# facebookresearch/AudioDec

Hardware: AMD Instinct MI355X
Metric: 48 kHz hop-300 frames/s/GPU + per-frame encode+decode latency (ms) (higher is better)
Workload: dtype f32 (conv operands split into f16 hi + lo/2048 pairs, 3 f16 MFMAs per product sum, f32 accumulate)

## Files before the change

### audiodec_amd/csrc/adk_common.h

```cpp
#pragma once
#include <hip/hip_runtime.h>
#include <stdint.h>
#include <string>
#include <algorithm>
#include <cstring>
#include <initializer_list>
#include "../../include/audiodec_hip.h"

namespace adk {

void set_error(const std::string& msg);
int fail(int code, const std::string& msg);

inline int check_pointers(const std::string& f, const char* names, bool missing, std::initializer_list<const void*> ptrs) {
    if (missing) return fail(ADK_ERR_ARG, f + ": null pointer");
    uintptr_t bits = 0;
    for (const void* p : ptrs) bits |= reinterpret_cast<uintptr_t>(p);
    if (bits & 3) return fail(ADK_ERR_ARG, f + ": " + names + " must be 4-byte aligned");
    return ADK_OK;
}

#define ADK_HIP_CHECK(expr)                                                                   \
    do {                                                                                      \
        hipError_t _e = (expr);                                                               \
        if (_e != hipSuccess)                                                                 \
            return ::adk::fail(ADK_ERR_HIP, std::string(#expr) + ": " + hipGetErrorString(_e)); \
    } while (0)

struct ConvArgs {
    const float* in;   int in_rows, in_ch, in_row0, in_choff, in_gstride;
    float* out;        int out_rows, out_ch, out_cursor, out_choff;
    const float* res;  int res_rows, res_ch, res_cursor, res_choff, res_gstride;
    const float* w;    const float* wfrag;  const float* bias;
    int cin_g, cout_g, groups, taps, stride, dilation, up, cout_real;
    int act_in, act_out; float slope;
    int batch, t_out, n_total;
    int ktot;
    int* err = nullptr;
    const float* in_sh = nullptr;
    float* out_sh = nullptr;
    int sh_act = 0; float sh_slope = 0.f;
};
inline int* conv_err_word(const ConvArgs& a);

__device__ __forceinline__ float expm1_neg(float x) {
    const float q = fmaf(fmaf(fmaf(fmaf(fmaf(1.f / 5040.f, x, 1.f / 720.f), x, 1.f / 120.f), x, 1.f / 24.f), x, 1.f / 6.f), x, 0.5f);
    const float p = fmaf(x * x, q, x);
    const float e = __builtin_amdgcn_exp2f(x * 1.44269504088896341f) - 1.0f;
    return x > -0.4f ? p : e;
}

__device__ __forceinline__ float act_apply(float x, int act, float slope) {
    if (act == ADK_ACT_ELU) return x > 0.f ? x : expm1_neg(x);
    if (act == ADK_ACT_LEAKY) return x > 0.f ? x : x * slope;
    if (act == ADK_ACT_TANH) return tanhf(x);
    return x;
}

__device__ __forceinline__ float rvq_residual_step(float& r, float q) {
    const float qp = __fadd_rn(r, __fsub_rn(q, r));
    r = __fsub_rn(r, qp);
    return qp;
}

struct RingMeanArgs {
    const float* src[4]; int src_rows[4], src_cursor[4];
    float* out; int out_rows, out_cursor;
    int n, channels, batch, t;
};
int launch_ring_mean(const RingMeanArgs& m, hipStream_t s);
int launch_hist_replicate(float* ring, int rows, int channels, int cursor, int hist, int batch, hipStream_t s);
int launch_conv_direct(const ConvArgs& a, hipStream_t s);
bool conv_cin1_write_ok(const ConvArgs& a);
int launch_conv_cin1_write(const ConvArgs& a, const float* src, hipStream_t s);
struct Workspace { float* ptr = nullptr; size_t bytes = 0; size_t flags_offset = 0; unsigned epoch = 0;
                   int workgroups = 0; };
int launch_conv_mfma(const ConvArgs& a, hipStream_t s, Workspace& ws);
size_t conv_mfma_workspace_bytes(size_t* flags_offset);
bool conv_rl_supported(const ConvArgs& a);
bool conv_rl_preferred(const ConvArgs& a);
int launch_conv_rl(const ConvArgs& a, hipStream_t s);
bool conv_rl16_supported(const ConvArgs& a);
bool conv_rl16_preferred(const ConvArgs& a);
int launch_conv_rl16(const ConvArgs& a, hipStream_t s);
bool conv_rl16_fusable(const ConvArgs& a1, const ConvArgs& a2);
int launch_conv_rl16_fused(const ConvArgs& a1, const ConvArgs& a2, hipStream_t s);
bool conv_rb16_fusable(const ConvArgs* c, int n);
int launch_conv_rb16(const ConvArgs* c, int n, const int* keep, hipStream_t s);
const char* conv_rb16_name(const ConvArgs* c, int n);
bool conv_ou16_fusable(const ConvArgs& a1, const ConvArgs& a2);
int launch_conv_ou16(const ConvArgs& a1, const ConvArgs& a2, hipStream_t s);
bool conv_oc16_fusable(const ConvArgs& a1, const ConvArgs& a2);
int launch_conv_oc16(const ConvArgs& a1, const ConvArgs& a2, hipStream_t s);
bool conv_up16_supported(const ConvArgs& a);
int launch_conv_up16(const ConvArgs& a, hipStream_t s);
int launch_conv_sk16(const ConvArgs& a, hipStream_t s, Workspace& ws);
int conv_sk16_pick(const ConvArgs& a);
bool conv_gv16_preferred(const ConvArgs& a);
int conv_set_option(const char* name, int value);
int rvq_set_option(const char* name, int value);
int rvq_ema_set_option(const char* name, int value);
int launch_pack_split16(const float* w, float* out, int groups, int cout_g, int ktot, hipStream_t s);
int* flags_word();
inline int* conv_err_word(const ConvArgs& a) { return a.err ? a.err : flags_word(); }
constexpr int kMaxDevices = 64;
int flag_pool_acquire(int device, int** word);
void flag_pool_release(int device, int* word);
int flag_pool_fetch(int device, int* word, hipStream_t s, int* v);
int flag_pool_take(int device, int* word, int* v);
int flag_pool_fetch_all(int device, int* acc);
inline int current_device() { int d = 0; (void)hipGetDevice(&d); return (d >= 0 && d < kMaxDevices) ? d : 0; }
inline int device_of(const void* ptr) {
    hipPointerAttribute_t at;
    if (ptr && hipPointerGetAttributes(&at, ptr) == hipSuccess && at.type == hipMemoryTypeDevice && at.device >= 0 && at.device < kMaxDevices)
        return at.device;
    (void)hipGetLastError();
    return current_device();
}
struct DeviceGuard {
    int prev = -1;
    explicit DeviceGuard(int device) {
        int cur = -1;
        if (hipGetDevice(&cur) == hipSuccess && cur != device) { if (hipSetDevice(device) == hipSuccess) prev = cur; }
    }
    ~DeviceGuard() { if (prev >= 0) (void)hipSetDevice(prev); }
};
int launch_pack_weights(const float* w, float* out, int groups, int cout_g, int ktot, hipStream_t s);
bool conv_mfma_supported(const ConvArgs& a);
int conv_mfma_pick(const ConvArgs& a);
const char* conv_mfma_cfg_name(int pick);
bool conv_mfma_force_cfg(int cfg);
int streamk_plan(long long tiles, int nchunks, int cap, int out[4]);
long long streamk_range_start(long long tiles, int nchunks, const int plan[4], int r);

}
```

### audiodec_amd/csrc/conv_mfma.hip

```cpp
#include "conv_split16.h"
#include <cstring>
#include <atomic>

#ifndef ADK_SK_SC1_READ
#define ADK_SK_SC1_READ 1
#endif
#ifndef ADK_SK_OWNER_LATE
#define ADK_SK_OWNER_LATE 1
#endif
#ifndef ADK_SK16_DBG
#define ADK_SK16_DBG 0
#endif

namespace adk {

#if ADK_SK16_DBG & 32
__device__ unsigned long long g_sk_wg_trace[512 * 4];
#endif
#if ADK_SK16_DBG & 16
__device__ unsigned long long g_sk_trace[64 * 8];
#define SK_STAMP(slot) do { if (trace_on && it < 64) { __builtin_amdgcn_sched_barrier(0); const unsigned long long t_ = __builtin_amdgcn_s_memtime(); \
                            __builtin_amdgcn_sched_barrier(0); if (lane == 0) trace_lds[it * 8 + (slot)] = t_; } } while (0)
#else
#define SK_STAMP(slot) do { } while (0)
#endif

constexpr int KC = 64;
constexpr int kGvCounters = 4096;

struct SkArgs {
    float* ws;
    unsigned* flags;
    unsigned epoch;
    int G;
    int split;
    int owner_chunks;
    int tpw;
    int tiles;
    int m_tiles, n_tiles, nchunks;
    int cpt;
    int kgroups;
    int mt32_per_g;
    unsigned in_bytes, w_bytes;
    unsigned ws_bytes;
    int* err;
    float inv_t_out;
    long long total;
    int epi_lds;
};

constexpr int kActPre = 100;

__host__ __device__ __forceinline__ long long sk_range_start(int r, int G, int split, int tpw, int tiles, int nchunks, int owner_chunks, long long total) {
    if (split > 0) {
        const int t = r / split, p = r - t * split;
        if (split == 2) return (long long)t * nchunks + (p ? owner_chunks : 0);
        return (long long)t * nchunks + (p * nchunks) / split;
    }
    if (tpw > 0) {
        long long t = (long long)r * tpw;
        if (t > tiles) t = tiles;
        return t * nchunks;
    }
    return (long long)r * total / G;
}
__device__ __forceinline__ long long sk_u0(int r, const SkArgs& sk) {
    return sk_range_start(r, sk.G, sk.split, sk.tpw, sk.tiles, sk.nchunks, sk.owner_chunks, sk.total);
}

template <int NJ, bool CHECK = false>
__device__ __forceinline__ void sk_epilogue(const ConvArgs& a, const f32x16 (&acc)[NJ], int g, int ml0, int n0w, int lane, int* err = nullptr) {
    const int l31 = lane & 31, lh = lane >> 5;
    bool bad = false;
#pragma unroll
    for (int j = 0; j < NJ; ++j) {
        const int n = n0w + j * 32 + l31;
        if (n >= a.n_total) continue;
        const int b = n / a.t_out, t = n - b * a.t_out;
        const float* resp = nullptr;
        if (a.res) {
            int rrow = a.res_cursor + t;
            if (rrow >= a.res_rows) rrow -= a.res_rows;
            resp = a.res + ((size_t)b * a.res_rows + rrow) * a.res_ch + a.res_choff + g * a.res_gstride;
        }
        float* outb = a.out + (size_t)b * a.out_rows * a.out_ch + a.out_choff;
        const int obase = a.out_cursor + t * a.up;
#pragma unroll
        for (int qd = 0; qd < 4; ++qd) {
            const int ml = ml0 + 8 * qd + 4 * lh;
            if (ml >= a.cout_g) continue;
            const int mg = g * a.cout_g + ml;
            float4 v = make_float4(acc[j][4 * qd], acc[j][4 * qd + 1], acc[j][4 * qd + 2], acc[j][4 * qd + 3]);
            if (CHECK) bad |= not_finite4(v);
            if (a.bias) {
                const float4 bb = *reinterpret_cast<const float4*>(a.bias + mg);
                v.x += bb.x; v.y += bb.y; v.z += bb.z; v.w += bb.w;
            }
            if (resp) {
                const float4 rr = *reinterpret_cast<const float4*>(resp + ml);
                v.x += rr.x; v.y += rr.y; v.z += rr.z; v.w += rr.w;
            }
            if (a.act_out != ADK_ACT_NONE) {
                v.x = act_apply(v.x, a.act_out, 0.f); v.y = act_apply(v.y, a.act_out, 0.f);
                v.z = act_apply(v.z, a.act_out, 0.f); v.w = act_apply(v.w, a.act_out, 0.f);
            }
            int orow = obase, ocol = mg;
            if (a.up > 1) { const int ph = mg / a.cout_real; orow += ph; ocol = mg - ph * a.cout_real; }
            if (orow >= a.out_rows) orow -= a.out_rows;
            *reinterpret_cast<float4*>(outb + (size_t)orow * a.out_ch + ocol) = v;
            if (CHECK && a.out_sh) {
                const float x[4] = {act_apply(v.x, a.sh_act, a.sh_slope), act_apply(v.y, a.sh_act, a.sh_slope),
                                    act_apply(v.z, a.sh_act, a.sh_slope), act_apply(v.w, a.sh_act, a.sh_slope)};
                f16x4 hi, lo;
#pragma unroll
                for (int e = 0; e < 4; ++e) split_to(x[e], hi, lo, e);
                unsigned char* srow = reinterpret_cast<unsigned char*>(a.out_sh + ((size_t)b * a.out_rows + orow) * a.out_ch + a.out_choff);
                unsigned char* sp = srow + (size_t)(ocol >> 3) * 32 + (ocol & 4) * 2;
                *reinterpret_cast<f16x4*>(sp) = hi;
                *reinterpret_cast<f16x4*>(sp + 16) = lo;
            }
        }
    }
    if (CHECK && bad) atomicOr(err, 8);
}

__device__ __forceinline__ void sk_tile_coords(int tile, const SkArgs& sk, int& g, int& mt, int& nt) {
    mt = tile % sk.m_tiles;
    const int rest = tile / sk.m_tiles;
    nt = rest % sk.n_tiles;
    g = rest / sk.n_tiles;
}

__device__ __forceinline__ int fast_div(int n, int d, float inv_d) {
    int q = (int)(__int2float_rn(n) * inv_d);
    int r = n - q * d;
    if (r < 0) { --q; r += d; }
    if (r >= d) { ++q; }
    return q;
}

template <int NJ, int BM, int BN, int NT, bool CHECK>
__device__ __forceinline__ void sk_epilogue_lds(const ConvArgs& a, const f32x16 (&acc)[NJ], float* T, int g, int m0, int n0, int wm, int wn,
                                                int tid, float inv_t_out, int* err) {
    constexpr int TSF = BM + 4;
    const int lane = tid & 63, l31 = lane & 31, lh = lane >> 5;
#pragma unroll
    for (int j = 0; j < NJ; ++j) {
        float* trow = T + (size_t)(wn * NJ * 32 + j * 32 + l31) * TSF + wm * 32 + 4 * lh;
#pragma unroll
        for (int qd = 0; qd < 4; ++qd)
            *reinterpret_cast<float4*>(trow + 8 * qd) = make_float4(acc[j][4 * qd], acc[j][4 * qd + 1], acc[j][4 * qd + 2], acc[j][4 * qd + 3]);
    }
    __syncthreads();
    constexpr int GPC = BM / 8;
    bool bad = false;
    for (int it = tid; it < BN * GPC; it += NT) {
        const int col = it / GPC, cg = it - col * GPC;
        const int n = n0 + col;
        const int ml = m0 + 8 * cg;
        if (n >= a.n_total || ml >= a.cout_g) continue;
        float4 t0 = *reinterpret_cast<const float4*>(T + (size_t)col * TSF + 8 * cg);
        float4 t1 = *reinterpret_cast<const float4*>(T + (size_t)col * TSF + 8 * cg + 4);
        if (CHECK) bad |= not_finite(t0.x) | not_finite(t0.y) | not_finite(t0.z) | not_finite(t0.w) |
                          not_finite(t1.x) | not_finite(t1.y) | not_finite(t1.z) | not_finite(t1.w);
        const int b = fast_div(n, a.t_out, inv_t_out), t = n - b * a.t_out;
        const int mg = g * a.cout_g + ml;
        if (a.bias) {
            const float4 b0 = *reinterpret_cast<const float4*>(a.bias + mg), b1 = *reinterpret_cast<const float4*>(a.bias + mg + 4);
            t0.x += b0.x; t0.y += b0.y; t0.z += b0.z; t0.w += b0.w;
            t1.x += b1.x; t1.y += b1.y; t1.z += b1.z; t1.w += b1.w;
        }
        if (a.res) {
            int rrow = a.res_cursor + t;
            if (rrow >= a.res_rows) rrow -= a.res_rows;
            const float* resp = a.res + ((size_t)b * a.res_rows + rrow) * a.res_ch + a.res_choff + g * a.res_gstride + ml;
            const float4 r0 = *reinterpret_cast<const float4*>(resp), r1 = *reinterpret_cast<const float4*>(resp + 4);
            t0.x += r0.x; t0.y += r0.y; t0.z += r0.z; t0.w += r0.w;
            t1.x += r1.x; t1.y += r1.y; t1.z += r1.z; t1.w += r1.w;
        }
        float x[8] = {t0.x, t0.y, t0.z, t0.w, t1.x, t1.y, t1.z, t1.w};
        if (a.act_out != ADK_ACT_NONE) {
#pragma unroll
            for (int e = 0; e < 8; ++e) x[e] = act_apply(x[e], a.act_out, 0.f);
        }
        int orow = a.out_cursor + t * a.up, ocol = mg;
        if (a.up > 1) { const int ph = mg / a.cout_real; orow += ph; ocol = mg - ph * a.cout_real; }
        if (orow >= a.out_rows) orow -= a.out_rows;
        const size_t oidx = ((size_t)b * a.out_rows + orow) * a.out_ch + a.out_choff + ocol;
        *reinterpret_cast<float4*>(a.out + oidx) = make_float4(x[0], x[1], x[2], x[3]);
        *reinterpret_cast<float4*>(a.out + oidx + 4) = make_float4(x[4], x[5], x[6], x[7]);
        if (CHECK && a.out_sh) {
            f16x8 hi, lo;
#pragma unroll
            for (int e = 0; e < 8; ++e) split_to(act_apply(x[e], a.sh_act, a.sh_slope), hi, lo, e);
            unsigned char* sp = reinterpret_cast<unsigned char*>(a.out_sh + ((size_t)b * a.out_rows + orow) * a.out_ch + a.out_choff) + (size_t)(ocol >> 3) * 32;
            *reinterpret_cast<f16x8*>(sp) = hi;
            *reinterpret_cast<f16x8*>(sp + 16) = lo;
        }
    }
    if (CHECK && bad) atomicOr(err, 8);
}

template <int WGM, int WGN, int NJ, int ACT, bool SPLIT, int KD>
__global__ __launch_bounds__(64 * WGM * WGN, (WGM * WGN == 4) ? 2 : 1) void conv_sk_kernel(ConvArgs a, SkArgs sk) {
    constexpr int NT = 64 * WGM * WGN;
    constexpr int BN = 32 * NJ * WGN;
    constexpr int KCC = KC * KD;
    constexpr int LDK = KCC + 4;
    constexpr int QPC = 16 * KD;
    constexpr int CPR = NT / QPC;
    constexpr int RB = BN / CPR;
    static_assert(WGM * WGN == 4 || WGM * WGN == 8, "4 or 8 waves");
    static_assert(BN % CPR == 0, "staging rounds");
    static_assert(SPLIT || KD == 1, "the exact-f32 variant keeps 64-deep chunks");
    extern __shared__ __attribute__((aligned(16))) float Bs[];

    const int tid = threadIdx.x, lane = tid & 63;
    const int wave = __builtin_amdgcn_readfirstlane(tid >> 6);
    const int wm = wave / WGN, wn = wave % WGN;
    const int l31 = lane & 31, lh = lane >> 5;
    const int srow = tid / QPC, quad = tid % QPC;
    const int half = quad >> 3;

    const int per_xcd = (sk.G + 7) >> 3;
    int r = (int)(blockIdx.x & 7) * per_xcd + (int)(blockIdx.x >> 3);
#if ADK_SK_OWNER_LATE
    if (sk.split == 2 && !(per_xcd & 1) && sk.G == 8 * per_xcd) {
        const int j = (int)(blockIdx.x >> 3), hp = per_xcd >> 1;
        r = (int)(blockIdx.x & 7) * per_xcd + (j < hp ? 2 * j + 1 : 2 * (j - hp));
    }
#endif
    if (r >= sk.G) return;
#if ADK_SK16_DBG & 32
    const unsigned long long wg_t0 = __builtin_amdgcn_s_memrealtime();
#endif
    const long long u0 = sk_u0(r, sk), u1 = sk_u0(r + 1, sk);
    if (u0 >= u1) return;

    const __amdgpu_buffer_rsrc_t rsrc_in = __builtin_amdgcn_make_buffer_rsrc(const_cast<float*>(a.in), 0, sk.in_bytes, 0x00020000);
    const __amdgpu_buffer_rsrc_t rsrc_w = __builtin_amdgcn_make_buffer_rsrc(const_cast<float*>(a.wfrag), 0, sk.w_bytes, 0x00020000);
    const unsigned row_bytes = (unsigned)a.in_ch * 4u;
    const unsigned ring_bytes = (unsigned)a.in_rows * row_bytes;
    const unsigned dil_bytes = (unsigned)a.dilation * row_bytes;
    const unsigned lane16 = (unsigned)lane * 16u;
    constexpr unsigned OOB = 0x80000000u;

    int s_tile, s_kc;
    int s_g = 0, s_mt = 0, s_nt = 0;
    int t_tap, t_cblk;
    unsigned colb[RB], rowb[RB];

    auto stage_tile = [&](int tile, int kc0) {
        sk_tile_coords(tile, sk, s_g, s_mt, s_nt);
        s_tile = tile; s_kc = kc0;
        const int j = 2 * KD * kc0 + half;
        t_tap = j / sk.cpt; t_cblk = j - t_tap * sk.cpt;
        const int n0 = s_nt * BN;
        const unsigned tap_bytes = (unsigned)t_tap * dil_bytes;
#pragma unroll
        for (int rr = 0; rr < RB; ++rr) {
            const int n = n0 + srow + CPR * rr;
            const int nn = n < a.n_total ? n : 0;
            const int b = fast_div(nn, a.t_out, sk.inv_t_out), t = nn - b * a.t_out;
            int row = a.in_row0 + t * a.stride;
            if (row >= a.in_rows) row -= a.in_rows;
            unsigned rbv = (unsigned)row * row_bytes + tap_bytes;
            if (rbv >= ring_bytes) rbv -= ring_bytes;
            rowb[rr] = rbv;
            colb[rr] = n < a.n_total ? ((unsigned)b * ring_bytes + (unsigned)(a.in_choff + s_g * a.in_gstride + 4 * (quad & 7)) * 4u) : OOB;
        }
    };
    auto stage_advance = [&]() {
        ++s_kc;
        if (s_kc == sk.nchunks) { stage_tile(s_tile + 1, 0); return; }
        t_cblk += 2 * KD;
        while (t_cblk >= sk.cpt) {
            t_cblk -= sk.cpt; ++t_tap;
#pragma unroll
            for (int rr = 0; rr < RB; ++rr) {
                unsigned rbv = rowb[rr] + dil_bytes;
                if (rbv >= ring_bytes) rbv -= ring_bytes;
                rowb[rr] = rbv;
            }
// ... 567 lines not shown
    }
    const unsigned grid = (unsigned)((sk.G + 7) / 8 * 8);
    if constexpr (SPLIT) {
        if (a.in_sh) {
            static bool pre_attr_dev[kMaxDevices] = {};
            bool& pre_attr = pre_attr_dev[current_device()];
            if (lds > 64 * 1024 && !pre_attr) {
                ADK_HIP_CHECK(hipFuncSetAttribute(reinterpret_cast<const void*>(conv_sk_kernel<WGM, WGN, NJ, kActPre, SPLIT, KD>), hipFuncAttributeMaxDynamicSharedMemorySize, (int)lds));
                pre_attr = true;
            }
            ConvArgs b = a;
            b.in = a.in_sh;
            hipLaunchKernelGGL((conv_sk_kernel<WGM, WGN, NJ, kActPre, SPLIT, KD>), dim3(grid), dim3(NT), lds, s, b, sk);
            ADK_HIP_CHECK(hipGetLastError());
            return ADK_OK;
        }
    }
    return with_act_in(a.act_in, "conv: unsupported input activation for the MFMA kernel", [&](auto act) -> int {
        hipLaunchKernelGGL((conv_sk_kernel<WGM, WGN, NJ, decltype(act)::value, SPLIT, KD>), dim3(grid), dim3(NT), lds, s, a, sk);
        ADK_HIP_CHECK(hipGetLastError());
        return ADK_OK;
    });
}
}

bool conv_mfma_force_cfg(int cfg) {
    if (cfg != -1 && cfg != 0 && cfg != 2 && cfg != 4) return false;
    g_forced_cfg = cfg;
    return true;
}

int streamk_plan(long long tiles, int nchunks, int cap, int out[4]) {
    SkArgs sk{};
    sk.nchunks = nchunks;
    const long long G = sk_plan(tiles, cap > 0 ? std::min<long long>(cap, kSlots) : kSlots, sk);
    out[0] = (int)G; out[1] = sk.split; out[2] = sk.tpw; out[3] = sk.owner_chunks;
    return ADK_OK;
}
long long streamk_range_start(long long tiles, int nchunks, const int plan[4], int r) {
    return sk_range_start(r, plan[0], plan[1], plan[2], (int)tiles, nchunks, plan[3], tiles * nchunks);
}

#if ADK_SK16_DBG & 32
extern "C" int adk_debug_sk_wg_trace(unsigned long long* out, int n) {
    if (n > 512 * 4) n = 512 * 4;
    return hipMemcpyFromSymbol(out, HIP_SYMBOL(g_sk_wg_trace), (size_t)n * sizeof(unsigned long long)) == hipSuccess ? 0 : -1;
}
#endif
#if ADK_SK16_DBG & 16
extern "C" int adk_debug_sk_trace(unsigned long long* out, int n) {
    if (n > 64 * 8) n = 64 * 8;
    return hipMemcpyFromSymbol(out, HIP_SYMBOL(g_sk_trace), (size_t)n * sizeof(unsigned long long)) == hipSuccess ? 0 : -1;
}
#endif

size_t conv_mfma_workspace_bytes(size_t* flags_offset) {
    const size_t part = (size_t)kSlots * 256 * 4 * 16 * sizeof(float);
    if (flags_offset) *flags_offset = part;
    return part + (size_t)kSlots * sizeof(unsigned)
           + (size_t)kGvCounters * sizeof(unsigned);
}

int conv_mfma_pick(const ConvArgs& a) {
    if (g_forced_cfg == 2 || g_forced_cfg == 4) return g_forced_cfg;
    return (a.cout_g % 64 == 0) ? 2 : 4;
}

const char* conv_mfma_cfg_name(int pick) { return kCfgs[pick].name; }

int launch_conv_mfma(const ConvArgs& a, hipStream_t s, Workspace& ws) {
    if (a.n_total == 0) return ADK_OK;
    return conv_mfma_pick(a) == 2 ? launch_cfg<2, 2, 1, false>(a, s, ws) : launch_cfg<1, 4, 1, false>(a, s, ws);
}

int conv_sk16_pick(const ConvArgs& a) {
    if (g_forced_cfg >= 0) return g_forced_cfg;
    if (a.cout_g % 128 == 0 && (long long)(a.cout_g / 128) * ((a.n_total + 63) / 64) * a.groups >= 256) return 0;
    return (a.cout_g % 64 == 0) ? 2 : 4;
}


static std::atomic<int> g_gv_maxn{32};
int conv_set_option(const char* name, int value) {
    if (strcmp(name, "gv16_max_columns")) return 1;
    g_gv_maxn.store(value < 0 ? 0 : value);
    return 0;
}
bool conv_gv16_preferred(const ConvArgs& a) {
    if (!conv_mfma_supported(a) || a.n_total < 1 || a.n_total > g_gv_maxn.load() || a.ktot % 16) return false;
    const long long steps = a.ktot / 16;
    const long long otiles = (long long)a.groups * ((a.cout_g + 31) / 32) * ((a.n_total + 31) / 32);
    if (steps > 15 * 24 || otiles > kGvCounters) return false;
    const long long S = steps <= 12 * 15 ? (steps + 11) / 12 : (steps + 23) / 24;
    size_t part = 0;
    (void)conv_mfma_workspace_bytes(&part);
    return otiles * S * 4096ll <= (long long)part && otiles * S <= 65535 * 8;
}

int launch_conv_gv16(const ConvArgs& a, hipStream_t s, Workspace& ws) {
    GvArgs gv;
    gv.mt32_per_g = (a.cout_g + 31) / 32;
    gv.tiles = a.groups * gv.mt32_per_g;
    gv.ntiles = (a.n_total + 31) / 32;
    gv.ksteps = a.ktot / 16;
    gv.ksteps_packed = (a.ktot + 63) / 64 * 4;
    gv.cpt16 = a.cin_g / 16;
    const bool small = gv.ksteps <= 12 * 15;
    gv.S = small ? (gv.ksteps + 11) / 12 : (gv.ksteps + 23) / 24;
    gv.inv_t_out = 1.0f / (float)a.t_out;
    gv.in_bytes = (unsigned)((unsigned long long)a.batch * a.in_rows * a.in_ch * 4ull);
    gv.w_bytes = (unsigned)((unsigned long long)a.groups * gv.mt32_per_g * gv.ksteps_packed * 2048ull);
    size_t flags_offset = 0;
    const size_t need = conv_mfma_workspace_bytes(&flags_offset);
    const size_t part = (size_t)gv.tiles * gv.ntiles * gv.S * 4096;
    if (!ws.ptr || ws.bytes < need || part > flags_offset) return fail(ADK_ERR_STATE, "conv_gv16: workspace missing or too small");
    gv.ws = ws.ptr; gv.ws_bytes = (unsigned)part;
    gv.counters = reinterpret_cast<unsigned*>(reinterpret_cast<char*>(ws.ptr) + need - (size_t)kGvCounters * sizeof(unsigned));
    gv.err = conv_err_word(a);
    const unsigned grid = (unsigned)(gv.tiles * gv.ntiles * gv.S);
    ConvArgs b = a;
    int act = a.act_in;
    if (a.in_sh) { b.in = a.in_sh; act = kActPre; }
    auto go = [&](auto act_c) -> int {
        constexpr int ACT = decltype(act_c)::value;
        if (small) hipLaunchKernelGGL((conv_gv16_kernel<ACT, 12>), dim3(grid), dim3(64), 0, s, b, gv);
        else hipLaunchKernelGGL((conv_gv16_kernel<ACT, 24>), dim3(grid), dim3(64), 0, s, b, gv);
        ADK_HIP_CHECK(hipGetLastError());
        return ADK_OK;
    };
    if (act == kActPre) return go(std::integral_constant<int, kActPre>());
    return with_act_in(act, "conv: unsupported input activation for the MFMA kernel", go);
}

int launch_conv_sk16(const ConvArgs& a, hipStream_t s, Workspace& ws) {
    if (a.n_total == 0) return ADK_OK;
    if (conv_gv16_preferred(a)) return launch_conv_gv16(a, s, ws);
    switch (conv_sk16_pick(a)) {
        case 0: return launch_cfg<4, 1, 2, true>(a, s, ws);
        case 2: return launch_cfg<2, 2, 1, true>(a, s, ws);
        default: return launch_cfg<1, 4, 1, true>(a, s, ws);
    }
}

int launch_pack_weights(const float* w, float* out, int groups, int cout_g, int ktot, hipStream_t s) {
    const long long total = (long long)groups * ((cout_g + 31) / 32) * ((ktot + 63) / 64 * 8) * 256;
    if (total == 0) return ADK_OK;
    long long blocks = (total + 255) / 256;
    if (blocks > 65535) blocks = 65535;
    hipLaunchKernelGGL(pack_weights_kernel, dim3((unsigned)blocks), dim3(256), 0, s, w, out, groups, cout_g, ktot);
    ADK_HIP_CHECK(hipGetLastError());
    return ADK_OK;
}

}
```

### audiodec_amd/csrc/program.hip

```cpp
#include "adk_common.h"
#include <vector>
#include <cstring>
#include <cstdio>
#include <cstdlib>
#include <mutex>
#include <atomic>

namespace adk {

static thread_local std::string g_err;
void set_error(const std::string& msg) { g_err = msg; }
int fail(int code, const std::string& msg) { g_err = msg; return code; }

static int build_args(const adk_conv_desc& d, const adk_ring_view& in, const adk_ring_view& out,
                      const adk_ring_view& res, int batch, int t_out, ConvArgs& a) {
    if ((!d.w && !d.w_frag) || !in.base || !out.base) return fail(ADK_ERR_ARG, "conv: null weight/in/out pointer");
    if (d.cin_g <= 0 || d.cout_g <= 0 || d.groups <= 0 || d.taps <= 0 || d.stride <= 0 || d.dilation <= 0 ||
        d.up <= 0 || d.cout_real <= 0 || d.hist < 0)
        return fail(ADK_ERR_SHAPE, "conv: non-positive geometry");
    if (batch < 0 || t_out < 0) return fail(ADK_ERR_SHAPE, "conv: negative batch / t_out");
    if ((long long)batch * t_out > 0x7fffffffLL) return fail(ADK_ERR_SHAPE, "conv: batch * t_out overflows");
    const long long M = (long long)d.groups * d.cout_g;
    if (M != (long long)d.up * d.cout_real) return fail(ADK_ERR_SHAPE, "conv: groups*cout_g != up*cout_real");
    if (d.up > 1 && d.groups != 1) return fail(ADK_ERR_SHAPE, "conv: transposed form needs groups == 1");
// ... 17 lines not shown
        return fail(ADK_ERR_ARG, "conv: unknown activation");
    a.in = in.base; a.in_rows = in.rows; a.in_ch = in.channels; a.in_choff = in.ch_off; a.in_gstride = d.in_group_stride;
    a.in_row0 = ((in.cursor - d.hist) % in.rows + in.rows) % in.rows;
    a.out = out.base; a.out_rows = out.rows; a.out_ch = out.channels; a.out_cursor = out.cursor; a.out_choff = out.ch_off;
    a.res = res.base; a.res_rows = res.rows; a.res_ch = res.channels; a.res_cursor = res.cursor; a.res_choff = res.ch_off;
    a.res_gstride = d.res_group_stride;
    a.w = d.w; a.wfrag = d.w_frag; a.bias = d.bias;
    a.cin_g = d.cin_g; a.cout_g = d.cout_g; a.groups = d.groups; a.taps = d.taps; a.stride = d.stride;
    a.dilation = d.dilation; a.up = d.up; a.cout_real = d.cout_real;
    a.act_in = d.act_in; a.act_out = d.act_out; a.slope = d.act_in_slope;
    a.batch = batch; a.t_out = t_out; a.n_total = batch * t_out; a.ktot = d.taps * d.cin_g;
    return ADK_OK;
}


static int ensure_workspace(Workspace& w) {
    size_t flags_offset = 0;
    const size_t need = conv_mfma_workspace_bytes(&flags_offset);
    if (w.ptr && w.bytes >= need) return ADK_OK;
    if (w.ptr) (void)hipFree(w.ptr);
    w.ptr = nullptr; w.bytes = 0;
    ADK_HIP_CHECK(hipMalloc(reinterpret_cast<void**>(&w.ptr), need));
    ADK_HIP_CHECK(hipMemset(w.ptr, 0, need));
    w.bytes = need; w.flags_offset = flags_offset; w.epoch = 0;
    return ADK_OK;
}

static std::atomic<int> g_use_chain{-1};
static std::atomic<int> g_chain_max_c{128};
static std::atomic<int> g_chain_min_blocks{0};
static std::atomic<int> g_use_ou{1};
static std::atomic<int> g_use_oc{1};
static std::atomic<int> g_use_cw{1};

static bool is_split16(int impl) {
    return impl == ADK_IMPL_SPLIT16 || impl == ADK_IMPL_SPLIT16_ROWS || impl == ADK_IMPL_SPLIT16_SK || impl == ADK_IMPL_SPLIT16_UP;
}
static bool chains_enabled() {
    if (g_use_chain < 0) { const char* e = getenv("ADK_CHAIN"); g_use_chain = e ? atoi(e) : 1; }
    return g_use_chain != 0;
}

static int run_conv(const ConvArgs& a, int impl, hipStream_t s, Workspace& ws) {
    const bool ok = conv_mfma_supported(a);
    if (impl == ADK_IMPL_MFMA_ROWS) {
        if (!conv_rl_supported(a)) return fail(ADK_ERR_SHAPE, "conv: rows-in-LDS kernel needs stride 1, 32/64 channels per group, w_frag");
        return launch_conv_rl(a, s);
    }
    if (a.out_sh && impl != ADK_IMPL_SPLIT16_SK)
        return fail(ADK_ERR_STATE, "conv: an op that writes a shadow ring must run on the split-f16 stream-K kernel (impl = ADK_IMPL_SPLIT16_SK)");
    if (is_split16(impl)) {
        if (impl == ADK_IMPL_SPLIT16_UP && !conv_up16_supported(a))
            return fail(ADK_ERR_SHAPE, "conv: the up-sampling streamer takes 2-tap transposed convs with 64 input channels and <= 96 GEMM rows");
        if (impl == ADK_IMPL_SPLIT16_UP || (impl == ADK_IMPL_SPLIT16 && conv_up16_supported(a)))
            return launch_conv_up16(a, s);
        if (impl == ADK_IMPL_SPLIT16_ROWS && !conv_rl16_supported(a))
            return fail(ADK_ERR_SHAPE, "conv: split-f16 rows-in-LDS kernel needs stride 1, 32/64 channels per group, K in {3,7,11}, split16 w_frag");
        if (impl == ADK_IMPL_SPLIT16_ROWS || (impl == ADK_IMPL_SPLIT16 && conv_rl16_preferred(a)))
            return launch_conv_rl16(a, s);
        if (!ok) return fail(ADK_ERR_SHAPE, "conv: split-f16 kernel needs w_frag, cin_g % 32 == 0 and 16-byte aligned rows");
        int rc = ensure_workspace(ws);
        if (rc != ADK_OK) return rc;
        return launch_conv_sk16(a, s, ws);
    }
    const bool want_mfma = (impl == ADK_IMPL_MFMA) || (impl == ADK_IMPL_AUTO && ok && a.groups * a.cout_g >= 32);
    if (impl == ADK_IMPL_MFMA && !ok)
        return fail(ADK_ERR_SHAPE, "conv: MFMA kernel needs w_frag, cin_g % 32 == 0 and 16-byte aligned rows");
    if (want_mfma) {
        if (impl == ADK_IMPL_AUTO && conv_rl_preferred(a)) return launch_conv_rl(a, s);
        int rc = ensure_workspace(ws);
        if (rc != ADK_OK) return rc;
        return launch_conv_mfma(a, s, ws);
    }
    if (!a.w) return fail(ADK_ERR_ARG, "conv: the VALU kernel needs row-major weights (w)");
    return launch_conv_direct(a, s);
}

static std::string conv_kernel_name(const ConvArgs& a, int impl) {
    if (is_split16(impl)) {
        if (impl == ADK_IMPL_SPLIT16_UP || (impl == ADK_IMPL_SPLIT16 && conv_up16_supported(a))) return "conv_up16<64>";
        const bool rows = impl == ADK_IMPL_SPLIT16_ROWS || (impl == ADK_IMPL_SPLIT16 && conv_rl16_preferred(a));
        if (rows) return a.cin_g == 32 ? "conv_rl16<32>" : "conv_rl16<64>";
        if (conv_gv16_preferred(a)) return "conv_gv16<32>";
        return std::string(conv_mfma_cfg_name(conv_sk16_pick(a))).replace(0, 7, "conv_sk16");
    }
    const bool mf = impl != ADK_IMPL_DIRECT && conv_mfma_supported(a) && (impl == ADK_IMPL_MFMA || impl == ADK_IMPL_MFMA_ROWS || a.groups * a.cout_g >= 32);
    const bool rl = mf && ((impl == ADK_IMPL_MFMA_ROWS && conv_rl_supported(a)) || (impl == ADK_IMPL_AUTO && conv_rl_preferred(a)));
    if (rl) return a.cin_g == 32 ? "conv_rl<32>" : "conv_rl<64>";
    if (mf) return conv_mfma_cfg_name(conv_mfma_pick(a));
    return a.groups * a.cout_g == 1 ? "conv_cout1" : (a.cin_g == 1 && a.taps == 7 ? "conv_cin1" : "conv_direct");
}

}

using namespace adk;

extern "C" const char* adk_last_error(void) { return g_err.c_str(); }
extern "C" int adk_abi_version(void) { return ADK_ABI_VERSION; }
extern "C" int adk_set_conv_cfg(int32_t cfg) {
    if (!conv_mfma_force_cfg(cfg)) return fail(ADK_ERR_ARG, "adk_set_conv_cfg: the library has tile configs 0 (128x64, split-f16 only), 2 (64x64) and 4 (32x128); -1 = heuristic");
    return ADK_OK;
}
extern "C" int adk_set_option(const char* name, int32_t value) {
    if (!name) return fail(ADK_ERR_ARG, "adk_set_option: null name");
    if (!strcmp(name, "chain_max_channels")) { g_chain_max_c = value < 0 ? 0 : value; return ADK_OK; }
    if (!strcmp(name, "chain_min_blocks")) { g_chain_min_blocks = value < 0 ? 0 : value; return ADK_OK; }
    if (!strcmp(name, "conv_ou16")) { g_use_ou = value != 0; return ADK_OK; }
    if (!strcmp(name, "conv_oc16")) { g_use_oc = value != 0; return ADK_OK; }
    if (!strcmp(name, "conv_cin1w")) { g_use_cw = value != 0; return ADK_OK; }
    if (conv_set_option(name, value) == 0) return ADK_OK;
    {
        const int r = rvq_set_option(name, value);
        if (r == 0) return ADK_OK;
        if (r < 0) return fail(ADK_ERR_ARG, std::string("adk_set_option: bad value for ") + name);
    }
    {
        const int r = rvq_ema_set_option(name, value);
        if (r == 0) return ADK_OK;
        if (r < 0) return fail(ADK_ERR_ARG, std::string("adk_set_option: bad value for ") + name);
    }
    return fail(ADK_ERR_ARG, std::string("adk_set_option: unknown option ") + name);
}

extern "C" int adk_streamk_plan(int64_t tiles, int32_t chunks, int32_t cap, int32_t* plan) {
    if (!plan || tiles < 1 || tiles >= (1ll << 31) / 64 || chunks < 1 || chunks > (1 << 20) || cap < 0) return fail(ADK_ERR_ARG, "adk_streamk_plan: bad argument");
    int out[4];
    const int rc = streamk_plan(tiles, chunks, cap, out);
    for (int i = 0; i < 4; ++i) plan[i] = out[i];
    return rc;
}

extern "C" int64_t adk_streamk_range_start(int64_t tiles, int32_t chunks, const int32_t* plan, int32_t r) {
    if (!plan || tiles < 1 || chunks < 1 || plan[0] < 1 || r < 0 || r > plan[0]) return -1;
    const int p[4] = {plan[0], plan[1], plan[2], plan[3]};
    return streamk_range_start(tiles, chunks, p, r);
}

extern "C" int adk_causal_conv(const adk_conv_desc* d, adk_ring_view in, adk_ring_view out, adk_ring_view res,
                               int32_t batch, int32_t t_out, int32_t impl, void* stream) {
    if (!d) return fail(ADK_ERR_ARG, "adk_causal_conv: null descriptor");
    ConvArgs a;
    int rc = build_args(*d, in, out, res, batch, t_out, a);
    if (rc != ADK_OK) return rc;
    DeviceGuard guard(device_of(out.base));
    static thread_local Workspace tls_ws[kMaxDevices];
    return run_conv(a, impl, static_cast<hipStream_t>(stream), tls_ws[current_device()]);
}

extern "C" int adk_causal_conv_describe(const adk_conv_desc* d, adk_ring_view in, adk_ring_view out, adk_ring_view res,
                                        int32_t batch, int32_t t_out, int32_t impl, char* buf, int32_t n) {
    if (!d || !buf || n <= 0) return fail(ADK_ERR_ARG, "adk_causal_conv_describe: null argument");
    ConvArgs a;
    int rc = build_args(*d, in, out, res, batch, t_out, a);
    if (rc != ADK_OK) return rc;
    snprintf(buf, n, "%s", conv_kernel_name(a, impl).c_str());
    return ADK_OK;
}

extern "C" int adk_causal_conv_time(const adk_conv_desc* d, adk_ring_view in, adk_ring_view out, adk_ring_view res,
                                    int32_t batch, int32_t t_out, int32_t impl, int32_t iters, void* stream, float* avg_us) {
    if (!d || !avg_us || iters <= 0) return fail(ADK_ERR_ARG, "adk_causal_conv_time: bad arguments");
    ConvArgs a;
    int rc = build_args(*d, in, out, res, batch, t_out, a);
    if (rc != ADK_OK) return rc;
    DeviceGuard guard(device_of(out.base));
    hipStream_t s = static_cast<hipStream_t>(stream);
// ... 640 lines not shown
```

Measured before the change: 283,000.

## Add row-staged split-f16 conv kernel reusing input rows across taps

Adds a new conv_rk16 kernel for stride-1 7/11-tap convs with cin_g>=128. It stages all input rows a 64-column tile needs into LDS once per 32-channel block and reads every tap from there, instead of re-fetching im2col columns per K step. The kernel splits K across two wave halves, reduces them through LDS, and prefetches weights per tap several units ahead. It is on by default for shapes that would otherwise take config 2 and have at least 192 tiles. The epilogue moves to a shared header. The cost is more LDS use, which may lower occupancy, plus the extra cross-wave reduction.

```diff
diff --git a/audiodec_amd/csrc/adk_common.h b/audiodec_amd/csrc/adk_common.h
--- a/audiodec_amd/csrc/adk_common.h
+++ b/audiodec_amd/csrc/adk_common.h
@@ -97,6 +97,10 @@
 int launch_conv_sk16(const ConvArgs& a, hipStream_t s, Workspace& ws);
 int conv_sk16_pick(const ConvArgs& a);
 bool conv_gv16_preferred(const ConvArgs& a);
+bool conv_rk16_eligible(const ConvArgs& a);
+bool conv_rk16_preferred(const ConvArgs& a);
+void conv_rk16_set(int value);
+int launch_conv_rk16(const ConvArgs& a, hipStream_t s);
 int conv_set_option(const char* name, int value);
 int rvq_set_option(const char* name, int value);
 int rvq_ema_set_option(const char* name, int value);
diff --git a/audiodec_amd/csrc/conv_mfma.hip b/audiodec_amd/csrc/conv_mfma.hip
--- a/audiodec_amd/csrc/conv_mfma.hip
+++ b/audiodec_amd/csrc/conv_mfma.hip
@@ -1,4 +1,4 @@
-#include "conv_split16.h"
+#include "conv_sk_epilogue.h"
 #include <cstring>
 #include <atomic>
 
@@ -49,7 +49,6 @@
     int epi_lds;
 };
 
-constexpr int kActPre = 100;
 
 __host__ __device__ __forceinline__ long long sk_range_start(int r, int G, int split, int tpw, int tiles, int nchunks, int owner_chunks, long long total) {
     if (split > 0) {
@@ -129,76 +128,6 @@
     const int rest = tile / sk.m_tiles;
     nt = rest % sk.n_tiles;
     g = rest / sk.n_tiles;
-}
-
-__device__ __forceinline__ int fast_div(int n, int d, float inv_d) {
-    int q = (int)(__int2float_rn(n) * inv_d);
-    int r = n - q * d;
-    if (r < 0) { --q; r += d; }
-    if (r >= d) { ++q; }
-    return q;
-}
-
-template <int NJ, int BM, int BN, int NT, bool CHECK>
-__device__ __forceinline__ void sk_epilogue_lds(const ConvArgs& a, const f32x16 (&acc)[NJ], float* T, int g, int m0, int n0, int wm, int wn,
-                                                int tid, float inv_t_out, int* err) {
-    constexpr int TSF = BM + 4;
-    const int lane = tid & 63, l31 = lane & 31, lh = lane >> 5;
-#pragma unroll
-    for (int j = 0; j < NJ; ++j) {
-        float* trow = T + (size_t)(wn * NJ * 32 + j * 32 + l31) * TSF + wm * 32 + 4 * lh;
-#pragma unroll
-        for (int qd = 0; qd < 4; ++qd)
-            *reinterpret_cast<float4*>(trow + 8 * qd) = make_float4(acc[j][4 * qd], acc[j][4 * qd + 1], acc[j][4 * qd + 2], acc[j][4 * qd + 3]);
-    }
-    __syncthreads();
-    constexpr int GPC = BM / 8;
-    bool bad = false;
-    for (int it = tid; it < BN * GPC; it += NT) {
-        const int col = it / GPC, cg = it - col * GPC;
-        const int n = n0 + col;
-        const int ml = m0 + 8 * cg;
-        if (n >= a.n_total || ml >= a.cout_g) continue;
-        float4 t0 = *reinterpret_cast<const float4*>(T + (size_t)col * TSF + 8 * cg);
-        float4 t1 = *reinterpret_cast<const float4*>(T + (size_t)col * TSF + 8 * cg + 4);
-        if (CHECK) bad |= not_finite(t0.x) | not_finite(t0.y) | not_finite(t0.z) | not_finite(t0.w) |
-                          not_finite(t1.x) | not_finite(t1.y) | not_finite(t1.z) | not_finite(t1.w);
-        const int b = fast_div(n, a.t_out, inv_t_out), t = n - b * a.t_out;
-        const int mg = g * a.cout_g + ml;
-        if (a.bias) {
-            const float4 b0 = *reinterpret_cast<const float4*>(a.bias + mg), b1 = *reinterpret_cast<const float4*>(a.bias + mg + 4);
-            t0.x += b0.x; t0.y += b0.y; t0.z += b0.z; t0.w += b0.w;
-            t1.x += b1.x; t1.y += b1.y; t1.z += b1.z; t1.w += b1.w;
-        }
-        if (a.res) {
-            int rrow = a.res_cursor + t;
-            if (rrow >= a.res_rows) rrow -= a.res_rows;
-            const float* resp = a.res + ((size_t)b * a.res_rows + rrow) * a.res_ch + a.res_choff + g * a.res_gstride + ml;
-            const float4 r0 = *reinterpret_cast<const float4*>(resp), r1 = *reinterpret_cast<const float4*>(resp + 4);
-            t0.x += r0.x; t0.y += r0.y; t0.z += r0.z; t0.w += r0.w;
-            t1.x += r1.x; t1.y += r1.y; t1.z += r1.z; t1.w += r1.w;
-        }
-        float x[8] = {t0.x, t0.y, t0.z, t0.w, t1.x, t1.y, t1.z, t1.w};
-        if (a.act_out != ADK_ACT_NONE) {
-#pragma unroll
-            for (int e = 0; e < 8; ++e) x[e] = act_apply(x[e], a.act_out, 0.f);
-        }
-        int orow = a.out_cursor + t * a.up, ocol = mg;
-        if (a.up > 1) { const int ph = mg / a.cout_real; orow += ph; ocol = mg - ph * a.cout_real; }
-        if (orow >= a.out_rows) orow -= a.out_rows;
-        const size_t oidx = ((size_t)b * a.out_rows + orow) * a.out_ch + a.out_choff + ocol;
-        *reinterpret_cast<float4*>(a.out + oidx) = make_float4(x[0], x[1], x[2], x[3]);
-        *reinterpret_cast<float4*>(a.out + oidx + 4) = make_float4(x[4], x[5], x[6], x[7]);
-        if (CHECK && a.out_sh) {
-            f16x8 hi, lo;
-#pragma unroll
-            for (int e = 0; e < 8; ++e) split_to(act_apply(x[e], a.sh_act, a.sh_slope), hi, lo, e);
-            unsigned char* sp = reinterpret_cast<unsigned char*>(a.out_sh + ((size_t)b * a.out_rows + orow) * a.out_ch + a.out_choff) + (size_t)(ocol >> 3) * 32;
-            *reinterpret_cast<f16x8*>(sp) = hi;
-            *reinterpret_cast<f16x8*>(sp + 16) = lo;
-        }
-    }
-    if (CHECK && bad) atomicOr(err, 8);
 }
 
 template <int WGM, int WGN, int NJ, int ACT, bool SPLIT, int KD>
@@ -932,6 +861,7 @@
 
 static std::atomic<int> g_gv_maxn{32};
 int conv_set_option(const char* name, int value) {
+    if (!strcmp(name, "conv_rk16")) { conv_rk16_set(value); return 0; }
     if (strcmp(name, "gv16_max_columns")) return 1;
     g_gv_maxn.store(value < 0 ? 0 : value);
     return 0;
@@ -985,6 +915,7 @@
 int launch_conv_sk16(const ConvArgs& a, hipStream_t s, Workspace& ws) {
     if (a.n_total == 0) return ADK_OK;
     if (conv_gv16_preferred(a)) return launch_conv_gv16(a, s, ws);
+    if (conv_rk16_preferred(a)) return launch_conv_rk16(a, s);
     switch (conv_sk16_pick(a)) {
         case 0: return launch_cfg<4, 1, 2, true>(a, s, ws);
         case 2: return launch_cfg<2, 2, 1, true>(a, s, ws);
diff --git a/audiodec_amd/csrc/conv_rk16.hip b/audiodec_amd/csrc/conv_rk16.hip
--- /dev/null
+++ b/audiodec_amd/csrc/conv_rk16.hip
@@ -0,0 +1,246 @@
+#include "conv_sk_epilogue.h"
+#include <atomic>
+#include <cstdlib>
+
+#ifndef ADK_RK16_PF11
+#define ADK_RK16_PF11 3
+#endif
+
+namespace adk {
+
+namespace {
+constexpr int kCB = 32;
+constexpr int kRS = 4 * kCB + 16;
+constexpr int kNT = 512;
+constexpr int kRounds = 4;
+constexpr int kMaxRows = 65536 / (2 * kRS);
+constexpr int kSumBytes = 2 * 4 * 64 * 64;
+constexpr int kEpiBytes = kSumBytes + 64 * (64 + 4) * 4;
+
+struct RkArgs {
+    int tiles, m_tiles, n_tiles;
+    int nblk;
+    int rps;
+    int nrows;
+    int ksteps;
+    int mt32_per_g;
+    unsigned in_bytes, w_bytes;
+    float inv_t_out;
+    int* err;
+};
+
+std::atomic<int> g_use_rk{-1};
+}
+
+template <int ACT, int TAPS>
+__global__ __launch_bounds__(kNT, 2) void conv_rk16_kernel(ConvArgs a, RkArgs rk) {
+    constexpr int PF = TAPS == 11 ? ADK_RK16_PF11 : 3, R = PF + 1;
+    static_assert(PF >= 1 && PF < TAPS, "the units in flight are those of one block");
+    constexpr unsigned OOB = 0x80000000u;
+    extern __shared__ __attribute__((aligned(16))) unsigned char xs[];
+
+    const int tid = threadIdx.x, lane = tid & 63;
+    const int wave = __builtin_amdgcn_readfirstlane(tid >> 6);
+    const int quad = wave & 3, kh = wave >> 2;
+    const int wm = quad >> 1, wn = quad & 1;
+    const int l31 = lane & 31, lh = lane >> 5;
+
+    const int per_xcd = (rk.tiles + 7) >> 3;
+    const int tile = (int)(blockIdx.x & 7) * per_xcd + (int)(blockIdx.x >> 3);
+    if (tile >= rk.tiles) return;
+    const int mt = tile % rk.m_tiles;
+    const int rest = tile / rk.m_tiles;
+    const int nt = rest % rk.n_tiles, g = rest / rk.n_tiles;
+    const int n0 = nt * 64, m0 = mt * 64;
+    const int b0 = n0 / a.t_out;
+    const int n_last = min(n0 + 63, a.n_total - 1);
+    const int rows_used = (n_last / a.t_out - b0 + 1) * rk.rps;
+
+    const __amdgpu_buffer_rsrc_t rsrc_in = __builtin_amdgcn_make_buffer_rsrc(const_cast<float*>(a.in), 0, rk.in_bytes, 0x00020000);
+    const __amdgpu_buffer_rsrc_t rsrc_w = __builtin_amdgcn_make_buffer_rsrc(const_cast<float*>(a.wfrag), 0, rk.w_bytes, 0x00020000);
+    const unsigned lane16 = (unsigned)lane * 16u;
+    const unsigned bufbytes = (unsigned)rk.nrows * kRS;
+
+    const int p = tid & 7;
+    unsigned goff[kRounds];
+    {
+        const unsigned row_bytes = (unsigned)a.in_ch * 4u, ring_bytes = (unsigned)a.in_rows * row_bytes;
+        const unsigned chan = (unsigned)(a.in_choff + g * a.in_gstride) * 4u + (unsigned)p * 16u;
+#pragma unroll
+        for (int k = 0; k < kRounds; ++k) {
+            const int row = (tid >> 3) + 64 * k;
+            goff[k] = OOB;
+            if (row < rows_used) {
+                const int sl = row / rk.rps, r = row - sl * rk.rps;
+                int rr = a.in_row0 + r;
+                if (rr >= a.in_rows) rr -= a.in_rows;
+                goff[k] = (unsigned)(b0 + sl) * ring_bytes + (unsigned)rr * row_bytes + chan;
+            }
+        }
+    }
+    const unsigned ldst0 = (unsigned)(tid >> 3) * kRS + (ACT == kActPre ? (unsigned)((p & 1) * 2 * kCB + (p >> 1) * 16) : (unsigned)(8 * p));
+    float4 sreg[kRounds];
+    auto gload = [&](int cb) {
+#pragma unroll
+        for (int k = 0; k < kRounds; ++k) sreg[k] = buf_load4(rsrc_in, goff[k] != OOB ? goff[k] + (unsigned)cb * (4u * kCB) : OOB, 0);
+    };
+    auto lstore = [&](int buf) {
+#pragma unroll
+        for (int k = 0; k < kRounds; ++k) {
+            if (goff[k] == OOB) continue;
+            unsigned char* d = xs + (unsigned)buf * bufbytes + ldst0 + (unsigned)k * (64 * kRS);
+            if constexpr (ACT == kActPre) {
+                *reinterpret_cast<float4*>(d) = sreg[k];
+            } else {
+                f16x4 hi, lo;
+                act_split4<ACT>(sreg[k], a.slope, hi, lo);
+                *reinterpret_cast<f16x4*>(d) = hi;
+                *reinterpret_cast<f16x4*>(d + 2 * kCB) = lo;
+            }
+        }
+    };
+
+    const unsigned wbase = (unsigned)((g * rk.mt32_per_g + mt * 2 + wm) * rk.ksteps + kh) * 2048u;
+    const unsigned tap_bytes = (unsigned)rk.nblk * 2u * 2048u;
+    u32x4 ah[R], al[R];
+
+    unsigned xoff;
+    {
+        const int nn = min(n0 + wn * 32 + l31, a.n_total - 1);
+        const int b = fast_div(nn, a.t_out, rk.inv_t_out), t = nn - b * a.t_out;
+        xoff = (unsigned)((b - b0) * rk.rps + t) * kRS + (unsigned)(kh * 32 + 16 * lh);
+    }
+    const unsigned dil_rs = (unsigned)a.dilation * kRS;
+
+    f32x16 acc[1], accx;
+#pragma unroll
+    for (int e = 0; e < 16; ++e) { acc[0][e] = 0.f; accx[e] = 0.f; }
+
+    gload(0);
+#pragma unroll
+    for (int i = 0; i < PF; ++i) {
+        ah[i] = __builtin_amdgcn_raw_buffer_load_b128(rsrc_w, lane16, wbase + (unsigned)i * tap_bytes, 0);
+        al[i] = __builtin_amdgcn_raw_buffer_load_b128(rsrc_w, lane16 + 1024u, wbase + (unsigned)i * tap_bytes, 0);
+    }
+    __builtin_amdgcn_sched_barrier(0);
+    lstore(0);
+    __syncthreads();
+
+    constexpr int P = (TAPS + R - 1) / R * R;
+    unsigned bufoff = 0;
+    auto block = [&](int cb, auto more) {
+        constexpr bool MORE = decltype(more)::value;
+        if constexpr (MORE) gload(cb + 1);
+        const unsigned wb = wbase + (unsigned)cb * 4096u;
+        const unsigned char* xb = xs + bufoff + xoff;
+#pragma unroll
+        for (int pos = 0; pos < P; ++pos) {
+            const int tpos = pos + PF, tj = tpos % P;
+            if (tj < TAPS && (tpos < P || MORE)) {
+                const unsigned so = wb + (tpos < P ? 0u : 4096u) + (unsigned)tj * tap_bytes;
+                ah[tj % R] = __builtin_amdgcn_raw_buffer_load_b128(rsrc_w, lane16, so, 0);
+                al[tj % R] = __builtin_amdgcn_raw_buffer_load_b128(rsrc_w, lane16 + 1024u, so, 0);
+            }
+            __builtin_amdgcn_sched_barrier(0);
+            if (pos < TAPS) {
+                const f16x8 bh = *reinterpret_cast<const f16x8*>(xb);
+                const f16x8 bl = *reinterpret_cast<const f16x8*>(xb + 2 * kCB);
+                xb += dil_rs;
+                const f16x8 Ah = as_f16x8(ah[pos % R]), Al = as_f16x8(al[pos % R]);
+                acc[0] = __builtin_amdgcn_mfma_f32_32x32x16_f16(Ah, bh, acc[0], 0, 0, 0);
+                accx = __builtin_amdgcn_mfma_f32_32x32x16_f16(Ah, bl, accx, 0, 0, 0);
+                accx = __builtin_amdgcn_mfma_f32_32x32x16_f16(Al, bh, accx, 0, 0, 0);
+            }
+        }
+        if constexpr (MORE) {
+            bufoff = bufbytes - bufoff;
+            lstore(bufoff ? 1 : 0);
+            __syncthreads();
+        }
+    };
+    for (int cb = 0; cb + 1 < rk.nblk; ++cb) block(cb, std::true_type());
+    block(rk.nblk - 1, std::false_type());
+
+#pragma unroll
+    for (int e = 0; e < 16; ++e) acc[0][e] = join(acc[0][e], accx[e]);
+    __syncthreads();
+    float4* S = reinterpret_cast<float4*>(xs);
+#pragma unroll
+    for (int e4 = 0; e4 < 4; ++e4)
+        S[((kh * 4 + quad) * 4 + e4) * 64 + lane] = make_float4(acc[0][4 * e4], acc[0][4 * e4 + 1], acc[0][4 * e4 + 2], acc[0][4 * e4 + 3]);
+    __syncthreads();
+#pragma unroll
+    for (int e4 = 0; e4 < 4; ++e4) {
+        const float4 o = S[(((kh ^ 1) * 4 + quad) * 4 + e4) * 64 + lane];
+        acc[0][4 * e4] += o.x; acc[0][4 * e4 + 1] += o.y; acc[0][4 * e4 + 2] += o.z; acc[0][4 * e4 + 3] += o.w;
+    }
+    sk_epilogue_lds<1, 64, 64, kNT, true>(a, acc, reinterpret_cast<float*>(xs + kSumBytes), g, m0, n0, wm, wn, tid, rk.inv_t_out, rk.err);
+}
+
+static int rk_tile_streams(const ConvArgs& a) {
+    const int s = (a.t_out - 1 + 63) / a.t_out + 1;
+    return std::min(s, a.batch);
+}
+
+bool conv_rk16_eligible(const ConvArgs& a) {
+    if (!conv_mfma_supported(a) || a.n_total < 1) return false;
+    if (a.stride != 1 || a.up != 1 || (a.taps != 7 && a.taps != 11)) return false;
+    if (a.cin_g < 128 || a.cin_g % 64 || a.cout_g % 64) return false;
+    if (conv_sk16_pick(a) != 2) return false;
+    if ((a.in_ch % 8) || (a.in_choff % 8) || (a.in_gstride % 8) || (a.out_ch % 8) || (a.out_choff % 8) || (a.cout_real % 8)) return false;
+    const long long rps = (long long)(a.taps - 1) * a.dilation + a.t_out;
+    if (rps > a.in_rows || 2 * rps > (long long)a.t_out * a.taps) return false;
+    if (rps * rk_tile_streams(a) > kMaxRows) return false;
+    return (long long)a.groups * (a.cout_g / 64) * ((a.n_total + 63) / 64) < (1ll << 28);
+}
+
+constexpr int kMinTiles = 192;
+
+bool conv_rk16_preferred(const ConvArgs& a) {
+    int on = g_use_rk.load();
+    if (on < 0) {
+        const char* e = getenv("ADK_CONV_RK16");
+        on = e ? atoi(e) : 1;
+        on = on < 0 ? 0 : (on > 2 ? 2 : on);
+        g_use_rk.store(on);
+    }
+    if (!on || !conv_rk16_eligible(a)) return false;
+    if (on == 2) return true;
+    if (a.groups > 1 && a.in_gstride == 0) return false;
+    return (long long)a.groups * (a.cout_g / 64) * ((a.n_total + 63) / 64) >= kMinTiles;
+}
+
+void conv_rk16_set(int value) { g_use_rk.store(value <= 0 ? 0 : (value > 2 ? 2 : value)); }
+
+int launch_conv_rk16(const ConvArgs& a, hipStream_t s) {
+    if (!conv_rk16_eligible(a)) return ADK_ERR_STATE;
+    RkArgs rk;
+    rk.m_tiles = a.cout_g / 64;
+    rk.n_tiles = (a.n_total + 63) / 64;
+    rk.tiles = a.groups * rk.m_tiles * rk.n_tiles;
+    rk.nblk = a.cin_g / kCB;
+    rk.rps = (a.taps - 1) * a.dilation + a.t_out;
+    rk.nrows = rk.rps * rk_tile_streams(a);
+    rk.ksteps = a.ktot / 16;
+    rk.mt32_per_g = a.cout_g / 32;
+    rk.in_bytes = (unsigned)((unsigned long long)a.batch * a.in_rows * a.in_ch * 4ull);
+    rk.w_bytes = (unsigned)((unsigned long long)a.groups * rk.mt32_per_g * rk.ksteps * 2048ull);
+    rk.inv_t_out = 1.0f / (float)a.t_out;
+    rk.err = conv_err_word(a);
+    const size_t lds = std::max<size_t>(2 * (size_t)rk.nrows * kRS, kEpiBytes);
+    const unsigned grid = (unsigned)((rk.tiles + 7) / 8 * 8);
+    ConvArgs b = a;
+    int act = a.act_in;
+    if (a.in_sh) { b.in = a.in_sh; act = kActPre; }
+    auto go = [&](auto act_c) -> int {
+        constexpr int ACT = decltype(act_c)::value;
+        if (a.taps == 7) hipLaunchKernelGGL((conv_rk16_kernel<ACT, 7>), dim3(grid), dim3(kNT), lds, s, b, rk);
+        else hipLaunchKernelGGL((conv_rk16_kernel<ACT, 11>), dim3(grid), dim3(kNT), lds, s, b, rk);
+        ADK_HIP_CHECK(hipGetLastError());
+        return ADK_OK;
+    };
+    if (act == kActPre) return go(std::integral_constant<int, kActPre>());
+    return with_act_in(act, "conv: unsupported input activation for the MFMA kernel", go);
+}
+
+}
diff --git a/audiodec_amd/csrc/conv_sk_epilogue.h b/audiodec_amd/csrc/conv_sk_epilogue.h
--- /dev/null
+++ b/audiodec_amd/csrc/conv_sk_epilogue.h
@@ -0,0 +1,78 @@
+#pragma once
+#include "conv_split16.h"
+
+namespace adk {
+
+constexpr int kActPre = 100;
+
+__device__ __forceinline__ int fast_div(int n, int d, float inv_d) {
+    int q = (int)(__int2float_rn(n) * inv_d);
+    int r = n - q * d;
+    if (r < 0) { --q; r += d; }
+    if (r >= d) { ++q; }
+    return q;
+}
+
+template <int NJ, int BM, int BN, int NT, bool CHECK>
+__device__ __forceinline__ void sk_epilogue_lds(const ConvArgs& a, const f32x16 (&acc)[NJ], float* T, int g, int m0, int n0, int wm, int wn,
+                                                int tid, float inv_t_out, int* err) {
+    constexpr int TSF = BM + 4;
+    const int lane = tid & 63, l31 = lane & 31, lh = lane >> 5;
+#pragma unroll
+    for (int j = 0; j < NJ; ++j) {
+        float* trow = T + (size_t)(wn * NJ * 32 + j * 32 + l31) * TSF + wm * 32 + 4 * lh;
+#pragma unroll
+        for (int qd = 0; qd < 4; ++qd)
+            *reinterpret_cast<float4*>(trow + 8 * qd) = make_float4(acc[j][4 * qd], acc[j][4 * qd + 1], acc[j][4 * qd + 2], acc[j][4 * qd + 3]);
+    }
+    __syncthreads();
+    constexpr int GPC = BM / 8;
+    bool bad = false;
+    for (int it = tid; it < BN * GPC; it += NT) {
+        const int col = it / GPC, cg = it - col * GPC;
+        const int n = n0 + col;
+        const int ml = m0 + 8 * cg;
+        if (n >= a.n_total || ml >= a.cout_g) continue;
+        float4 t0 = *reinterpret_cast<const float4*>(T + (size_t)col * TSF + 8 * cg);
+        float4 t1 = *reinterpret_cast<const float4*>(T + (size_t)col * TSF + 8 * cg + 4);
+        if (CHECK) bad |= not_finite(t0.x) | not_finite(t0.y) | not_finite(t0.z) | not_finite(t0.w) |
+                          not_finite(t1.x) | not_finite(t1.y) | not_finite(t1.z) | not_finite(t1.w);
+        const int b = fast_div(n, a.t_out, inv_t_out), t = n - b * a.t_out;
+        const int mg = g * a.cout_g + ml;
+        if (a.bias) {
+            const float4 b0 = *reinterpret_cast<const float4*>(a.bias + mg), b1 = *reinterpret_cast<const float4*>(a.bias + mg + 4);
+            t0.x += b0.x; t0.y += b0.y; t0.z += b0.z; t0.w += b0.w;
+            t1.x += b1.x; t1.y += b1.y; t1.z += b1.z; t1.w += b1.w;
+        }
+        if (a.res) {
+            int rrow = a.res_cursor + t;
+            if (rrow >= a.res_rows) rrow -= a.res_rows;
+            const float* resp = a.res + ((size_t)b * a.res_rows + rrow) * a.res_ch + a.res_choff + g * a.res_gstride + ml;
+            const float4 r0 = *reinterpret_cast<const float4*>(resp), r1 = *reinterpret_cast<const float4*>(resp + 4);
+            t0.x += r0.x; t0.y += r0.y; t0.z += r0.z; t0.w += r0.w;
+            t1.x += r1.x; t1.y += r1.y; t1.z += r1.z; t1.w += r1.w;
+        }
+        float x[8] = {t0.x, t0.y, t0.z, t0.w, t1.x, t1.y, t1.z, t1.w};
+        if (a.act_out != ADK_ACT_NONE) {
+#pragma unroll
+            for (int e = 0; e < 8; ++e) x[e] = act_apply(x[e], a.act_out, 0.f);
+        }
+        int orow = a.out_cursor + t * a.up, ocol = mg;
+        if (a.up > 1) { const int ph = mg / a.cout_real; orow += ph; ocol = mg - ph * a.cout_real; }
+        if (orow >= a.out_rows) orow -= a.out_rows;
+        const size_t oidx = ((size_t)b * a.out_rows + orow) * a.out_ch + a.out_choff + ocol;
+        *reinterpret_cast<float4*>(a.out + oidx) = make_float4(x[0], x[1], x[2], x[3]);
+        *reinterpret_cast<float4*>(a.out + oidx + 4) = make_float4(x[4], x[5], x[6], x[7]);
+        if (CHECK && a.out_sh) {
+            f16x8 hi, lo;
+#pragma unroll
+            for (int e = 0; e < 8; ++e) split_to(act_apply(x[e], a.sh_act, a.sh_slope), hi, lo, e);
+            unsigned char* sp = reinterpret_cast<unsigned char*>(a.out_sh + ((size_t)b * a.out_rows + orow) * a.out_ch + a.out_choff) + (size_t)(ocol >> 3) * 32;
+            *reinterpret_cast<f16x8*>(sp) = hi;
+            *reinterpret_cast<f16x8*>(sp + 16) = lo;
+        }
+    }
+    if (CHECK && bad) atomicOr(err, 8);
+}
+
+}
diff --git a/audiodec_amd/csrc/program.hip b/audiodec_amd/csrc/program.hip
--- a/audiodec_amd/csrc/program.hip
+++ b/audiodec_amd/csrc/program.hip
@@ -123,6 +123,7 @@
         const bool rows = impl == ADK_IMPL_SPLIT16_ROWS || (impl == ADK_IMPL_SPLIT16 && conv_rl16_preferred(a));
         if (rows) return a.cin_g == 32 ? "conv_rl16<32>" : "conv_rl16<64>";
         if (conv_gv16_preferred(a)) return "conv_gv16<32>";
+        if (conv_rk16_preferred(a)) return "conv_sk16<rk16 64x64>";
         return std::string(conv_mfma_cfg_name(conv_sk16_pick(a))).replace(0, 7, "conv_sk16");
     }
     const bool mf = impl != ADK_IMPL_DIRECT && conv_mfma_supported(a) && (impl == ADK_IMPL_MFMA || impl == ADK_IMPL_MFMA_ROWS || a.groups * a.cout_g >= 32);
```

New measurement: 290,800 (median of 6 runs). 1.03x the previous value.
